# apple/ml-fastvlm

Measured on AMD Instinct MI355X. Metric: images/sec FastViTHD encode_images @1024x1024 bf16, higher is better.
Workload: dtype bf16; 1 GPU; BASELINE.json configs[1]: FastViTHD encoder + mlp2x_gelu projector (H=896), batch=32/GPU synthetic 1024x1024 bf16 images in [0,1), seeded synthetic weights, single GPU; global_batch=32, image_size=1024, parallelism=dp1, hip_graph=False, attention_operands=bf16, ffn_precision=auto (calibrated on the benchmark batch), range guard on

## Files before the change

ml_fastvlm_amd/csrc/attention.hip:

```cpp
#include "fvhd_common.h"
#include "launchers.h"

template <int VPL>
__global__ __launch_bounds__(256) void layernorm_kernel(const bf16* __restrict__ x, bf16* __restrict__ y,
                                                        const float* __restrict__ w, const float* __restrict__ b,
                                                        int M, int C, float eps)
{
    const int lane = threadIdx.x & 63;
    const int row = blockIdx.x * 4 + (threadIdx.x >> 6);
    if (row >= M) return;
    const bf16* xr = x + (size_t)row * C;
    f32x4 v[VPL];
    float s = 0.f;
#pragma unroll
    for (int i = 0; i < VPL; ++i) {
        const int c = (i * 64 + lane) * 4;
        if (c < C) {
            v[i] = bf4_to_f32(*(const bf16x4*)(xr + c));
            s += v[i][0] + v[i][1] + v[i][2] + v[i][3];
        } else v[i] = f32x4{0.f, 0.f, 0.f, 0.f};
    }
    const float mean = wave_sum(s) / (float)C;
    float q = 0.f;
#pragma unroll
    for (int i = 0; i < VPL; ++i) {
        const int c = (i * 64 + lane) * 4;
        if (c < C) {
#pragma unroll
            for (int k = 0; k < 4; ++k) { const float d = v[i][k] - mean; q += d * d; }
        }
    }
    const float rstd = 1.0f / sqrtf(wave_sum(q) / (float)C + eps);
    bf16* yr = y + (size_t)row * C;
#pragma unroll
    for (int i = 0; i < VPL; ++i) {
        const int c = (i * 64 + lane) * 4;
        if (c < C) {
            const f32x4 wv = *(const f32x4*)(w + c), bv = *(const f32x4*)(b + c);
            f32x4 o;
#pragma unroll
            for (int k = 0; k < 4; ++k) o[k] = (v[i][k] - mean) * rstd * wv[k] + bv[k];
            *(bf16x4*)(yr + c) = f32_to_bf4(o);
        }
    }
}

extern "C" int fvhd_launch_layernorm(hipStream_t st, const void* x, void* y, const float* w, const float* b,
                                     int M, int C, float eps)
{
    if (C % 4 || C > 256 * 8) return (int)hipErrorInvalidValue;
    const int vpl = (C + 255) / 256;
    dim3 grid((M + 3) / 4), block(256);
    const bf16* xi = (const bf16*)x;
    bf16* yo = (bf16*)y;
#define LN_CASE(V) case V: hipLaunchKernelGGL((layernorm_kernel<V>), grid, block, 0, st, xi, yo, w, b, M, C, eps); break;
    switch (vpl) { LN_CASE(1) LN_CASE(2) LN_CASE(3) LN_CASE(4) LN_CASE(5) LN_CASE(6) LN_CASE(7) LN_CASE(8) }
#undef LN_CASE
    return (int)hipGetLastError();
}

#define ATT_D 32
#define ATT_KT 64
#ifndef ATT_QW
#define ATT_QW 2
#endif
#define ATT_QB (64 * ATT_QW)
#ifndef ATT_VTR
#define ATT_VTR 1
#endif
typedef short att_s16x4 __attribute__((ext_vector_type(4)));
typedef __attribute__((address_space(3))) att_s16x4* att_lds_s16x4p;
#define ATT_VT_STRIDE 136

FVHD_DEV long pack_fp8x8(f32x8 v)
{
#pragma unroll
    for (int i = 0; i < 8; ++i) v[i] = (v[i] != v[i]) ? v[i] : __builtin_amdgcn_fmed3f(v[i], -448.0f, 448.0f);
    int lo = __builtin_amdgcn_cvt_pk_fp8_f32(v[0], v[1], 0, false);
    lo = __builtin_amdgcn_cvt_pk_fp8_f32(v[2], v[3], lo, true);
    int hi = __builtin_amdgcn_cvt_pk_fp8_f32(v[4], v[5], 0, false);
    hi = __builtin_amdgcn_cvt_pk_fp8_f32(v[6], v[7], hi, true);
    return (long)(((unsigned long)(unsigned)hi << 32) | (unsigned)lo);
}
#define ATT_VT8_STRIDE 68

template <bool FP8>
__global__ __launch_bounds__(256) void attention_kernel(const bf16* __restrict__ qkv, bf16* __restrict__ out,
                                                        int N, int C, float scale_log2e)
{
    __shared__ __attribute__((aligned(16))) char lds[2 * (ATT_KT * 64 + ATT_D * ATT_VT_STRIDE)];
    const int tid = threadIdx.x, lane = tid & 63, wave = tid >> 6;
    const int lr = lane & 15, g = lane >> 4;
    const int nqb = (N + ATT_QB - 1) / ATT_QB, nh = C / ATT_D;
    const int L = xcd_remap(blockIdx.x, gridDim.x);
    const int qb = L % nqb, h = (L / nqb) % nh, b = L / (nqb * nh);
    const size_t row_stride = (size_t)3 * C;
    const bf16* base = qkv + (size_t)b * N * row_stride + h * ATT_D;

    int q_idx[ATT_QW];
    bf16x8 qf[ATT_QW];
    long qf8[ATT_QW];
#pragma unroll
    for (int w = 0; w < ATT_QW; ++w) {
        q_idx[w] = qb * ATT_QB + (wave * ATT_QW + w) * 16 + lr;
        qf[w] = *(const bf16x8*)(base + (size_t)min(q_idx[w], N - 1) * row_stride + g * 8);
        if constexpr (FP8) qf8[w] = pack_fp8x8(bf8_to_f32(qf[w]));
    }

    const int skey = tid >> 2, sch = tid & 3;
    const bf16* kptr = base + C + sch * 8;
    const bf16* vptr = base + 2 * C + sch * 8;
    const int k_dst = skey * 64 + ((sch ^ ((0 - (skey >> 2)) & 3)) << 4);
    const int k8_dst = skey * 32 + ((sch ^ (((skey >> 3) & 1) << 1)) << 3);
    const int v_dst = skey * 64 + ((sch ^ (((skey >> 2) & 1) << 1)) << 4);
    const unsigned v_src = lds_addr(lds) + (unsigned)(ATT_KT * 64 + (4 * g + (lr >> 2)) * 64 + (lr & 3) * 8);

    f32x4 o_acc[ATT_QW][2];
    f32x4 l_acc[ATT_QW];
    float m_run[ATT_QW];
    bf16x8 ones;
    const long ones8 = 0x3838383838383838L;
#pragma unroll
    for (int i = 0; i < 8; ++i) ones[i] = (bf16)1.0f;
#pragma unroll
    for (int w = 0; w < ATT_QW; ++w) {
        o_acc[w][0] = f32x4{0.f, 0.f, 0.f, 0.f};
        o_acc[w][1] = f32x4{0.f, 0.f, 0.f, 0.f};
        l_acc[w] = f32x4{0.f, 0.f, 0.f, 0.f};
        m_run[w] = -1e30f;
    }

    const int ntiles = (N + ATT_KT - 1) / ATT_KT;
    u32x4 rk, rv;
    const bf16* kcur = kptr + (size_t)min(skey, N - 1) * row_stride;
    const bf16* vcur = vptr + (size_t)min(skey, N - 1) * row_stride;
    const size_t tile_step = (size_t)ATT_KT * row_stride;
    rk = *(const u32x4*)kcur;
    rv = *(const u32x4*)vcur;
    for (int t = 0; t < ntiles; ++t) {
        char* kbuf = lds + (t & 1) * (ATT_KT * 64 + ATT_D * ATT_VT_STRIDE);
        char* vbuf = kbuf + ATT_KT * 64;
        if constexpr (FP8) {
            *(long*)(kbuf + k8_dst) = pack_fp8x8(bf8_to_f32(__builtin_bit_cast(bf16x8, rk)));
            const long v8 = pack_fp8x8(bf8_to_f32(__builtin_bit_cast(bf16x8, rv)));
#pragma unroll
            for (int i = 0; i < 8; ++i) *(unsigned char*)(vbuf + (sch * 8 + i) * ATT_VT8_STRIDE + skey) = (unsigned char)(v8 >> (8 * i));
        } else {
            *(u32x4*)(kbuf + k_dst) = rk;
#if ATT_VTR
            *(u32x4*)(vbuf + v_dst) = rv;
#else
            const bf16x8 vv = __builtin_bit_cast(bf16x8, rv);
#pragma unroll
            for (int i = 0; i < 8; ++i) *(bf16*)(vbuf + (sch * 8 + i) * ATT_VT_STRIDE + skey * 2) = vv[i];
#endif
        }
        __syncthreads();
        if (t + 1 < ntiles) {
            if ((t + 2) * ATT_KT <= N) {
                kcur += tile_step;
                vcur += tile_step;
            } else {
                const int key = min((t + 1) * ATT_KT + skey, N - 1);
                kcur = kptr + (size_t)key * row_stride;
                vcur = vptr + (size_t)key * row_stride;
            }
            rk = *(const u32x4*)kcur;
            rv = *(const u32x4*)vcur;
        }

        f32x4 s[ATT_QW][4];
#pragma unroll
        for (int kf = 0; kf < 4; ++kf) {
            const int krow = kf * 16 + lr;
            if constexpr (FP8) {
                const long kfr = *(const long*)(kbuf + krow * 32 + ((g ^ (((krow >> 3) & 1) << 1)) << 3));
#pragma unroll
                for (int w = 0; w < ATT_QW; ++w)
                    s[w][kf] = __builtin_amdgcn_mfma_f32_16x16x32_fp8_fp8(kfr, qf8[w], f32x4{0.f, 0.f, 0.f, 0.f}, 0, 0, 0);
            } else {
                const bf16x8 kfr = *(const bf16x8*)(kbuf + krow * 64 + ((g ^ ((0 - (krow >> 2)) & 3)) << 4));
#pragma unroll
                for (int w = 0; w < ATT_QW; ++w)
                    s[w][kf] = __builtin_amdgcn_mfma_f32_16x16x32_bf16(kfr, qf[w], f32x4{0.f, 0.f, 0.f, 0.f}, 0, 0, 0);
            }
        }
        if ((t + 1) * ATT_KT > N) {
            asm volatile("; ragged key tile");
#pragma unroll
            for (int w = 0; w < ATT_QW; ++w)
#pragma unroll
                for (int kf = 0; kf < 4; ++kf)
#pragma unroll
                    for (int r = 0; r < 4; ++r)
                        if (t * ATT_KT + kf * 16 + g * 4 + r >= N) s[w][kf][r] = -1e30f;
        }
        long pf8[ATT_QW][2];
        bf16x8 pf[ATT_QW][2];
#pragma unroll
        for (int w = 0; w < ATT_QW; ++w) {
            float mx = -1e30f;
#pragma unroll
            for (int kf = 0; kf < 4; ++kf)
#pragma unroll
                for (int r = 0; r < 4; ++r) mx = fmaxf(mx, s[w][kf][r]);
            mx = fmaxf(mx, __shfl_xor(mx, 16, 64));
            mx = fmaxf(mx, __shfl_xor(mx, 32, 64));
            const float m_new = fmaxf(m_run[w], mx);
            const float alpha = __builtin_amdgcn_exp2f((m_run[w] - m_new) * scale_log2e);
            m_run[w] = m_new;
            const float mb = m_new * scale_log2e;
#pragma unroll
            for (int c = 0; c < 2; ++c) {
                f32x8 p;
#pragma unroll
                for (int r = 0; r < 4; ++r) {
                    p[r] = __builtin_amdgcn_exp2f(__builtin_fmaf(s[w][2 * c][r], scale_log2e, -mb));
                    p[4 + r] = __builtin_amdgcn_exp2f(__builtin_fmaf(s[w][2 * c + 1][r], scale_log2e, -mb));
                }
                if constexpr (FP8) pf8[w][c] = pack_fp8x8(p);
                else pf[w][c] = f32_to_bf8(p);
            }
            if (__builtin_amdgcn_ballot_w64(alpha != 1.0f) != 0) {
                l_acc[w] *= alpha;
                o_acc[w][0] *= alpha;
                o_acc[w][1] *= alpha;
            }
#pragma unroll
            for (int c = 0; c < 2; ++c) {
                if constexpr (FP8) l_acc[w] = __builtin_amdgcn_mfma_f32_16x16x32_fp8_fp8(ones8, pf8[w][c], l_acc[w], 0, 0, 0);
                else l_acc[w] = __builtin_amdgcn_mfma_f32_16x16x32_bf16(ones, pf[w][c], l_acc[w], 0, 0, 0);
            }
        }
#pragma unroll
        for (int df = 0; df < 2; ++df)
#pragma unroll
            for (int c = 0; c < 2; ++c) {
                if constexpr (FP8) {
                    const char* vr = vbuf + (df * 16 + lr) * ATT_VT8_STRIDE + c * 32 + g * 4;
                    const unsigned lo = *(const unsigned*)(vr), hi = *(const unsigned*)(vr + 16);
                    const long vf = (long)(((unsigned long)hi << 32) | lo);
#pragma unroll
                    for (int w = 0; w < ATT_QW; ++w)
                        o_acc[w][df] = __builtin_amdgcn_mfma_f32_16x16x32_fp8_fp8(vf, pf8[w][c], o_acc[w][df], 0, 0, 0);
                } else {
#if ATT_VTR
                    const unsigned va = v_src + (unsigned)((t & 1) * (ATT_KT * 64 + ATT_D * ATT_VT_STRIDE) + c * 32 * 64) + (unsigned)((df ^ (g & 1)) << 5);
                    const att_s16x4 lo4 = __builtin_amdgcn_ds_read_tr16_b64_v4i16((att_lds_s16x4p)(size_t)va);
                    const att_s16x4 hi4 = __builtin_amdgcn_ds_read_tr16_b64_v4i16((att_lds_s16x4p)(size_t)(va + 16 * 64));
                    const bf16x4 lo = __builtin_bit_cast(bf16x4, lo4), hi = __builtin_bit_cast(bf16x4, hi4);
                    const bf16x8 vf = __builtin_shufflevector(lo, hi, 0, 1, 2, 3, 4, 5, 6, 7);
#else
                    const char* vr = vbuf + (df * 16 + lr) * ATT_VT_STRIDE + (c * 32 + g * 4) * 2;
                    const bf16x4 lo = *(const bf16x4*)(vr);
                    const bf16x4 hi = *(const bf16x4*)(vr + 32);
                    const bf16x8 vf = __builtin_shufflevector(lo, hi, 0, 1, 2, 3, 4, 5, 6, 7);
#endif
#pragma unroll
                    for (int w = 0; w < ATT_QW; ++w)
                        o_acc[w][df] = __builtin_amdgcn_mfma_f32_16x16x32_bf16(vf, pf[w][c], o_acc[w][df], 0, 0, 0);
                }
            }
    }

#pragma unroll
    for (int w = 0; w < ATT_QW; ++w)
        if (q_idx[w] < N) {
            const float inv = 1.0f / l_acc[w][0];
            bf16* orow = out + ((size_t)b * N + q_idx[w]) * C + h * ATT_D;
#pragma unroll
            for (int df = 0; df < 2; ++df)
                *(bf16x4*)(orow + df * 16 + g * 4) = f32_to_bf4(o_acc[w][df] * inv);
        }
}

extern "C" int fvhd_launch_attention(hipStream_t st, const void* qkv, void* out, int B, int N, int C, int fp8)
{
    if (C % ATT_D || B <= 0 || N <= 0) return (int)hipErrorInvalidValue;
    dim3 grid((unsigned)(((N + ATT_QB - 1) / ATT_QB) * (C / ATT_D) * B));
    const float scale_log2e = 0.17677669529663687f * 1.4426950408889634f;
    if (fp8) hipLaunchKernelGGL(attention_kernel<true>, grid, dim3(256), 0, st, (const bf16*)qkv, (bf16*)out, N, C, scale_log2e);
    else hipLaunchKernelGGL(attention_kernel<false>, grid, dim3(256), 0, st, (const bf16*)qkv, (bf16*)out, N, C, scale_log2e);
    return (int)hipGetLastError();
}
```

Before: 1443 images/sec.

## Load K/V tiles straight into LDS via global_load_lds DMA in attention

In the bf16 path, K and V tiles now go from global memory directly into LDS with global_load_lds_dwordx4, issued through inline asm that sets m0. This replaces the load-to-register then ds_write staging, and the swizzle moves into the source column offsets. The tile loop is unrolled by two with compile-time buffer parity, K-fragment and V-transpose addresses are hoisted, and the row max uses three-input max chains. The risks are correctness of the m0/vmcnt handling in inline asm, and that each wave writes contiguous 1KB chunks, so the swizzled layout depends on the DMA lane mapping.

Result: no change. 1446 images/sec (median of 3 runs) (+0.2%).

```diff
diff --git a/ml_fastvlm_amd/csrc/attention.hip b/ml_fastvlm_amd/csrc/attention.hip
--- a/ml_fastvlm_amd/csrc/attention.hip
+++ b/ml_fastvlm_amd/csrc/attention.hip
@@ -1,3 +1,5 @@
+#include <type_traits>
+
 #include "fvhd_common.h"
 #include "launchers.h"
 
@@ -65,12 +67,25 @@
 #define ATT_QW 2
 #endif
 #define ATT_QB (64 * ATT_QW)
-#ifndef ATT_VTR
-#define ATT_VTR 1
-#endif
 typedef short att_s16x4 __attribute__((ext_vector_type(4)));
 typedef __attribute__((address_space(3))) att_s16x4* att_lds_s16x4p;
 #define ATT_VT_STRIDE 136
+#define ATT_BUF (ATT_KT * 64 + ATT_D * ATT_VT_STRIDE)
+
+FVHD_DEV void att_dma_kv(const void* sbase, unsigned koff, unsigned voff, unsigned kdst, unsigned vdst)
+{
+    unsigned keep;
+    asm volatile("s_mov_b32 %0, m0\n\ts_mov_b32 m0, %4\n\ts_nop 0\n\tglobal_load_lds_dwordx4 %1, %3\n\t"
+                 "s_mov_b32 m0, %5\n\ts_nop 0\n\tglobal_load_lds_dwordx4 %2, %3\n\ts_mov_b32 m0, %0"
+                 : "=&s"(keep) : "v"(koff), "v"(voff), "s"(sbase), "s"(kdst), "s"(vdst) : "memory");
+}
+#ifndef ATT_U2
+#define ATT_U2 1
+#endif
+template <int P> FVHD_DEV constexpr int att_par(std::integral_constant<int, P>) { return P; }
+FVHD_DEV constexpr int att_par(int p) { return p; }
+FVHD_DEV void att_wait_dma() { asm volatile("s_waitcnt vmcnt(0)" ::: "memory"); }
+FVHD_DEV float att_max3(float a, float b, float c) { return fmaxf(fmaxf(a, b), c); }
 
 FVHD_DEV long pack_fp8x8(f32x8 v)
 {
@@ -88,8 +103,8 @@
 __global__ __launch_bounds__(256) void attention_kernel(const bf16* __restrict__ qkv, bf16* __restrict__ out,
                                                         int N, int C, float scale_log2e)
 {
-    __shared__ __attribute__((aligned(16))) char lds[2 * (ATT_KT * 64 + ATT_D * ATT_VT_STRIDE)];
-    const int tid = threadIdx.x, lane = tid & 63, wave = tid >> 6;
+    __shared__ __attribute__((aligned(16))) char lds[2 * ATT_BUF];
+    const int tid = threadIdx.x, lane = tid & 63, wave = __builtin_amdgcn_readfirstlane(tid >> 6);
     const int lr = lane & 15, g = lane >> 4;
     const int nqb = (N + ATT_QB - 1) / ATT_QB, nh = C / ATT_D;
     const int L = xcd_remap(blockIdx.x, gridDim.x);
@@ -108,12 +123,18 @@
     }
 
     const int skey = tid >> 2, sch = tid & 3;
-    const bf16* kptr = base + C + sch * 8;
-    const bf16* vptr = base + 2 * C + sch * 8;
-    const int k_dst = skey * 64 + ((sch ^ ((0 - (skey >> 2)) & 3)) << 4);
+    const int kch = FP8 ? sch : sch ^ ((0 - (skey >> 2)) & 3);
+    const int vch = FP8 ? sch : sch ^ (((skey >> 2) & 1) << 1);
+    const unsigned row_bytes = 6u * (unsigned)C, kcol = 2u * (unsigned)(C + kch * 8), vcol = 2u * (unsigned)(2 * C + vch * 8);
+    const unsigned koff = (unsigned)min(skey, N - 1) * row_bytes + kcol, voff = (unsigned)min(skey, N - 1) * row_bytes + vcol;
+    const size_t tile_step = (size_t)ATT_KT * row_bytes;
     const int k8_dst = skey * 32 + ((sch ^ (((skey >> 3) & 1) << 1)) << 3);
-    const int v_dst = skey * 64 + ((sch ^ (((skey >> 2) & 1) << 1)) << 4);
-    const unsigned v_src = lds_addr(lds) + (unsigned)(ATT_KT * 64 + (4 * g + (lr >> 2)) * 64 + (lr & 3) * 8);
+    const int kf_base = FP8 ? lr * 32 + ((g ^ (((lr >> 3) & 1) << 1)) << 3) : lr * 64 + ((g ^ ((0 - (lr >> 2)) & 3)) << 4);
+    unsigned v_src[2];
+#pragma unroll
+    for (int df = 0; df < 2; ++df)
+        v_src[df] = lds_addr(lds) + (unsigned)(ATT_KT * 64 + (4 * g + (lr >> 2)) * 64 + (lr & 3) * 8) + (unsigned)((df ^ (g & 1)) << 5);
+    const unsigned dma_dst = lds_addr(lds) + (unsigned)wave * 1024u;
 
     f32x4 o_acc[ATT_QW][2];
     f32x4 l_acc[ATT_QW];
@@ -132,13 +153,27 @@
 
     const int ntiles = (N + ATT_KT - 1) / ATT_KT;
     u32x4 rk, rv;
-    const bf16* kcur = kptr + (size_t)min(skey, N - 1) * row_stride;
-    const bf16* vcur = vptr + (size_t)min(skey, N - 1) * row_stride;
-    const size_t tile_step = (size_t)ATT_KT * row_stride;
-    rk = *(const u32x4*)kcur;
-    rv = *(const u32x4*)vcur;
-    for (int t = 0; t < ntiles; ++t) {
-        char* kbuf = lds + (t & 1) * (ATT_KT * 64 + ATT_D * ATT_VT_STRIDE);
+    const char* sb = (const char*)base;
+    auto fetch = [&](int tn, int par) {
+        unsigned ko = koff, vo = voff;
+        if ((tn + 1) * ATT_KT > N) {
+            const unsigned key = (unsigned)min(skey, N - 1 - tn * ATT_KT);
+            ko = key * row_bytes + kcol;
+            vo = key * row_bytes + vcol;
+        }
+        if constexpr (FP8) {
+            rk = *(const u32x4*)(sb + ko);
+            rv = *(const u32x4*)(sb + vo);
+        } else {
+            const unsigned kd = dma_dst + (unsigned)par * ATT_BUF;
+            att_dma_kv(sb, ko, vo, kd, kd + ATT_KT * 64);
+        }
+    };
+    fetch(0, 0);
+    if constexpr (!FP8) asm volatile("" :: "v"(qf[0]), "v"(qf[ATT_QW - 1]));
+    auto tile = [&](int t, auto parc) {
+        const int par = att_par(parc);
+        char* kbuf = lds + par * ATT_BUF;
         char* vbuf = kbuf + ATT_KT * 64;
         if constexpr (FP8) {
             *(long*)(kbuf + k8_dst) = pack_fp8x8(bf8_to_f32(__builtin_bit_cast(bf16x8, rk)));
@@ -146,40 +181,24 @@
 #pragma unroll
             for (int i = 0; i < 8; ++i) *(unsigned char*)(vbuf + (sch * 8 + i) * ATT_VT8_STRIDE + skey) = (unsigned char)(v8 >> (8 * i));
         } else {
-            *(u32x4*)(kbuf + k_dst) = rk;
-#if ATT_VTR
-            *(u32x4*)(vbuf + v_dst) = rv;
-#else
-            const bf16x8 vv = __builtin_bit_cast(bf16x8, rv);
-#pragma unroll
-            for (int i = 0; i < 8; ++i) *(bf16*)(vbuf + (sch * 8 + i) * ATT_VT_STRIDE + skey * 2) = vv[i];
-#endif
+            att_wait_dma();
         }
         __syncthreads();
         if (t + 1 < ntiles) {
-            if ((t + 2) * ATT_KT <= N) {
-                kcur += tile_step;
-                vcur += tile_step;
-            } else {
-                const int key = min((t + 1) * ATT_KT + skey, N - 1);
-                kcur = kptr + (size_t)key * row_stride;
-                vcur = vptr + (size_t)key * row_stride;
-            }
-            rk = *(const u32x4*)kcur;
-            rv = *(const u32x4*)vcur;
+            sb += tile_step;
+            fetch(t + 1, par ^ 1);
         }
 
         f32x4 s[ATT_QW][4];
 #pragma unroll
         for (int kf = 0; kf < 4; ++kf) {
-            const int krow = kf * 16 + lr;
             if constexpr (FP8) {
-                const long kfr = *(const long*)(kbuf + krow * 32 + ((g ^ (((krow >> 3) & 1) << 1)) << 3));
+                const long kfr = *(const long*)(kbuf + kf_base + kf * 16 * 32);
 #pragma unroll
                 for (int w = 0; w < ATT_QW; ++w)
                     s[w][kf] = __builtin_amdgcn_mfma_f32_16x16x32_fp8_fp8(kfr, qf8[w], f32x4{0.f, 0.f, 0.f, 0.f}, 0, 0, 0);
             } else {
-                const bf16x8 kfr = *(const bf16x8*)(kbuf + krow * 64 + ((g ^ ((0 - (krow >> 2)) & 3)) << 4));
+                const bf16x8 kfr = *(const bf16x8*)(kbuf + kf_base + kf * 16 * 64);
 #pragma unroll
                 for (int w = 0; w < ATT_QW; ++w)
                     s[w][kf] = __builtin_amdgcn_mfma_f32_16x16x32_bf16(kfr, qf[w], f32x4{0.f, 0.f, 0.f, 0.f}, 0, 0, 0);
@@ -199,11 +218,14 @@
         bf16x8 pf[ATT_QW][2];
 #pragma unroll
         for (int w = 0; w < ATT_QW; ++w) {
-            float mx = -1e30f;
-#pragma unroll
-            for (int kf = 0; kf < 4; ++kf)
-#pragma unroll
-                for (int r = 0; r < 4; ++r) mx = fmaxf(mx, s[w][kf][r]);
+            float mx = att_max3(s[w][0][0], s[w][0][1], s[w][0][2]);
+            mx = att_max3(mx, s[w][0][3], s[w][1][0]);
+            mx = att_max3(mx, s[w][1][1], s[w][1][2]);
+            mx = att_max3(mx, s[w][1][3], s[w][2][0]);
+            mx = att_max3(mx, s[w][2][1], s[w][2][2]);
+            mx = att_max3(mx, s[w][2][3], s[w][3][0]);
+            mx = att_max3(mx, s[w][3][1], s[w][3][2]);
+            mx = fmaxf(mx, s[w][3][3]);
             mx = fmaxf(mx, __shfl_xor(mx, 16, 64));
             mx = fmaxf(mx, __shfl_xor(mx, 32, 64));
             const float m_new = fmaxf(m_run[w], mx);
@@ -244,24 +266,27 @@
                     for (int w = 0; w < ATT_QW; ++w)
                         o_acc[w][df] = __builtin_amdgcn_mfma_f32_16x16x32_fp8_fp8(vf, pf8[w][c], o_acc[w][df], 0, 0, 0);
                 } else {
-#if ATT_VTR
-                    const unsigned va = v_src + (unsigned)((t & 1) * (ATT_KT * 64 + ATT_D * ATT_VT_STRIDE) + c * 32 * 64) + (unsigned)((df ^ (g & 1)) << 5);
+                    const unsigned va = v_src[df] + (unsigned)(par * ATT_BUF + c * 32 * 64);
                     const att_s16x4 lo4 = __builtin_amdgcn_ds_read_tr16_b64_v4i16((att_lds_s16x4p)(size_t)va);
                     const att_s16x4 hi4 = __builtin_amdgcn_ds_read_tr16_b64_v4i16((att_lds_s16x4p)(size_t)(va + 16 * 64));
                     const bf16x4 lo = __builtin_bit_cast(bf16x4, lo4), hi = __builtin_bit_cast(bf16x4, hi4);
                     const bf16x8 vf = __builtin_shufflevector(lo, hi, 0, 1, 2, 3, 4, 5, 6, 7);
-#else
-                    const char* vr = vbuf + (df * 16 + lr) * ATT_VT_STRIDE + (c * 32 + g * 4) * 2;
-                    const bf16x4 lo = *(const bf16x4*)(vr);
-                    const bf16x4 hi = *(const bf16x4*)(vr + 32);
-                    const bf16x8 vf = __builtin_shufflevector(lo, hi, 0, 1, 2, 3, 4, 5, 6, 7);
-#endif
 #pragma unroll
                     for (int w = 0; w < ATT_QW; ++w)
                         o_acc[w][df] = __builtin_amdgcn_mfma_f32_16x16x32_bf16(vf, pf[w][c], o_acc[w][df], 0, 0, 0);
                 }
             }
-    }
+    };
+#if ATT_U2
+    int t = 0;
+    for (; t + 1 < ntiles; t += 2) {
+        tile(t, std::integral_constant<int, 0>{});
+        tile(t + 1, std::integral_constant<int, 1>{});
+    }
+    if (t < ntiles) tile(t, std::integral_constant<int, 0>{});
+#else
+    for (int t = 0; t < ntiles; ++t) tile(t, t & 1);
+#endif
 
 #pragma unroll
     for (int w = 0; w < ATT_QW; ++w)
```
